# KoslickiLab/YACHT

Measured on AMD Instinct MI355X. Metric: ref-sketch containment queries/sec (yacht run), higher is better.
Workload: dtype u64

## Files before the change

### yacht_amd/csrc/yh_query.hip

```cpp
#include "yh_lookup.h"

#include <stdlib.h>
#include <string.h>

#include <algorithm>
#include <vector>

namespace {

constexpr int WAVE = 64;
constexpr int EXCL_PIECE_C = YH_EXCL_PIECE;

typedef u64 u64x2 __attribute__((ext_vector_type(2)));

__device__ __forceinline__ u32 xcd_remap(u32 bid, u32 nwg) {
    const u32 q = nwg >> 3, r = nwg & 7u;
    const u32 xcd = bid & 7u;
    const u32 base = (xcd < r) ? xcd * (q + 1) : r * (q + 1) + (xcd - r) * q;
    return base + (bid >> 3);
}

#ifndef YH_XCD_ATOMICS
#define YH_XCD_ATOMICS 0
#endif
__device__ __forceinline__ u32 xcc_id() { return (u32)__builtin_amdgcn_s_getreg((3 << 11) | 20) & 7u; }
__device__ __forceinline__ void count_add(u32* p, u32 v) {
#if YH_XCD_ATOMICS
    __hip_atomic_fetch_add(p, v, __ATOMIC_RELAXED, __HIP_MEMORY_SCOPE_WORKGROUP);
#else
    atomicAdd(p, v);
#endif
}
__device__ __forceinline__ u32 replica_of(u32 wg, u32 rep_mask) {
#if YH_XCD_ATOMICS
    return xcc_id() & rep_mask;
#else
    return wg & rep_mask;
#endif
}

struct FusedRun {
    u32* reps2;
    const u32* sizes;
    const u32* nshared;
    u32* n_excl;
    u32* n_match;
    u32* bits_out;
    const u32* rpo;
    uint4* work;
    u32* work_count;
    u32 work_refs;
};

__device__ __forceinline__ void append_pieces(bool in_subset, u32 j, u32 nshared_j, u32 rpo_j, uint4* __restrict__ work,
                                              u32* __restrict__ work_count, u32* lds ) {
    const u32 lane = threadIdx.x & 63u, wv = threadIdx.x >> 6, n_waves = blockDim.x >> 6;
    const u32 np = in_subset ? (nshared_j + (u32)EXCL_PIECE_C - 1u) / (u32)EXCL_PIECE_C : 0u;
    u32 v = np;
#pragma unroll
    for (int off = 1; off < 64; off <<= 1) {
        const u32 t = (u32)__shfl_up((int)v, off);
        if (lane >= (u32)off) v += t;
    }
    if (lane == 63) lds[wv] = v;
    __syncthreads();
    if (threadIdx.x == 0) {
        u32 total = 0;
        for (u32 q = 0; q < n_waves; ++q) total += lds[q];
        lds[n_waves] = total ? atomicAdd(work_count, total) : 0u;
    }
    __syncthreads();
    u32 at = lds[n_waves] + v - np;
    for (u32 q = 0; q < wv; ++q) at += lds[q];
    const u32 last = rpo_j + nshared_j;
    for (u32 i = 0; i < np; ++i) {
        const u32 first = rpo_j + i * (u32)EXCL_PIECE_C;
        work[at + i] = make_uint4(j, first, min(first + (u32)EXCL_PIECE_C, last), 0u);
    }
}

__device__ __forceinline__ void reduce_replicas_body(u32 wg, u32* lds, u32* __restrict__ reps, u32 R, u64 n,
                                                     u32* __restrict__ out, u8* __restrict__ mask,
                                                     u32* __restrict__ maskbits, u32* __restrict__ excl3,
                                                     const FusedRun& fused) {
    const u64 j = wg * (u64)blockDim.x + threadIdx.x;
    u32 acc = 0;
    u32 size_j = 0, nshared_j = 0, rpo_j = 0, rpo_end = 0;
    if (j < n && fused.reps2) {
        size_j = fused.sizes[j];
        nshared_j = fused.nshared[j];
        if (fused.work) { rpo_j = fused.rpo[j]; rpo_end = fused.rpo[j + 1]; }
    }
    if (j < n) {
        for (u32 r = 0; r < R; ++r) {
            acc += reps[(u64)r * n + j];
            reps[(u64)r * n + j] = 0;
        }
        out[j] = acc;
        if (mask) mask[j] = acc ? 1 : 0;
        if (excl3) { excl3[j] = 0; excl3[n + j] = 0; excl3[2 * n + j] = 0; }
        if (fused.reps2) {
            u32 acc2 = 0;
            for (u32 r = 0; r < R; ++r) {
                acc2 += fused.reps2[(u64)r * n + j];
                fused.reps2[(u64)r * n + j] = 0;
            }
            fused.n_match[j] = acc - acc2;
            if (fused.n_excl) fused.n_excl[j] = acc ? size_j - nshared_j : 0u;
        }
    }
    if (maskbits) {
        const u64 bal = __ballot(acc != 0);
        if ((threadIdx.x & 63) == 0 && (j >> 5) < ((n + 255) / 256) * 8) {
            maskbits[(j >> 5)] = (u32)bal;
            maskbits[(j >> 5) + 1] = (u32)(bal >> 32);
            if (fused.bits_out) {
                fused.bits_out[(j >> 5)] = (u32)bal;
                fused.bits_out[(j >> 5) + 1] = (u32)(bal >> 32);
            }
        }
    }
    if (fused.work) append_pieces(acc != 0 && j < fused.work_refs, (u32)j, rpo_end - rpo_j, rpo_j, fused.work, fused.work_count, lds);
}

__global__ void __launch_bounds__(256) k_reduce_replicas(u32* __restrict__ reps, u32 R, u64 n,
                                                         u32* __restrict__ out, u8* __restrict__ mask,
                                                         u32* __restrict__ maskbits, u32* __restrict__ excl3,
                                                         FusedRun fused) {
    __shared__ u32 lds[17];
    reduce_replicas_body(blockIdx.x, lds, reps, R, n, out, mask, maskbits, excl3, fused);
}

constexpr int FUSED_MAX_REPS = 16;
constexpr u32 FUSED_REPS_FORM1 = 8, FUSED_REPS_FORM2 = 8;
__device__ __forceinline__ u32 word_at(const u32* base, u32 byte_off) {
    return *reinterpret_cast<const u32*>(reinterpret_cast<const char*>(base) + byte_off);
}
template <int RPT, int G>
__device__ __forceinline__ void sum_replica_rows(const u32* set, u32 R, u64 n, const u32 (&off)[RPT], const bool (&ok)[RPT],
                                                 u32 (&acc)[RPT]) {
#pragma unroll 1
    for (u32 g = 0; g < R; g += (u32)G) {
        u32 t[RPT][G];
#pragma unroll
        for (u32 k = 0; k < (u32)G; ++k) {
            const u64 row = (u64)min(g + k, R - 1u) * n;
#pragma unroll
            for (int r = 0; r < RPT; ++r) t[r][k] = word_at(set + row, off[r]);
        }
#pragma unroll
        for (u32 k = 0; k < (u32)G; ++k)
#pragma unroll
            for (int r = 0; r < RPT; ++r) acc[r] += t[r][k] & ((ok[r] && g + k < R) ? ~0u : 0u);
    }
}
template <int RPT>
__device__ __forceinline__ void reduce_replicas_multi(u32 blk, u32* lds, u32* __restrict__ reps, u32 R, u64 n, u32* __restrict__ out,
                                                      u32* __restrict__ maskbits, const FusedRun& f) {
    const u32 lane = threadIdx.x & 63u, wv = threadIdx.x >> 6, n_waves = blockDim.x >> 6;
    const u64 j0 = (u64)blk * RPT * blockDim.x + threadIdx.x;
    u32 jj[RPT], off[RPT];
    bool ok[RPT];
    u32 acc[RPT], acc2[RPT], size_j[RPT], nsh[RPT], rpo0[RPT], rpo1[RPT];
#pragma unroll
    for (int r = 0; r < RPT; ++r) {
        ok[r] = j0 + (u64)r * blockDim.x < n;
        jj[r] = (u32)min(j0 + (u64)r * blockDim.x, n - 1);
        off[r] = jj[r] * 4u;
        acc[r] = acc2[r] = size_j[r] = nsh[r] = rpo0[r] = rpo1[r] = 0;
    }
    if (R >= 8u) sum_replica_rows<RPT, 8>(reps, R, n, off, ok, acc);
    else sum_replica_rows<RPT, 4>(reps, R, n, off, ok, acc);
#pragma unroll
    for (int r = 0; r < RPT; ++r) {
        if (acc[r]) {
            const u32 off1[1] = {off[r]};
            const bool ok1[1] = {true};
            u32 a2[1] = {0u};
            size_j[r] = f.sizes[jj[r]];
            nsh[r] = f.nshared[jj[r]];
            rpo0[r] = f.work ? f.rpo[jj[r]] : 0u;
            rpo1[r] = f.work ? f.rpo[jj[r] + 1u] : 0u;
            sum_replica_rows<1, 8>(f.reps2, R, n, off1, ok1, a2);
            acc2[r] = a2[0];
            for (u32 k = 0; k < R; ++k) (reps + (u64)k * n)[jj[r]] = 0;
            if (acc2[r])
                for (u32 k = 0; k < R; ++k) (f.reps2 + (u64)k * n)[jj[r]] = 0;
        }
    }
#pragma unroll
    for (int r = 0; r < RPT; ++r) {
        if (ok[r]) {
            out[jj[r]] = acc[r];
            f.n_match[jj[r]] = acc[r] - acc2[r];
            if (f.n_excl) f.n_excl[jj[r]] = acc[r] ? size_j[r] - nsh[r] : 0u;
        }
        const u64 bal = __ballot(acc[r] != 0);
        const u64 jr = j0 + (u64)r * blockDim.x;
        if (lane == 0 && (jr >> 5) < ((n + 255) / 256) * 8) {
            maskbits[(jr >> 5)] = (u32)bal;
            maskbits[(jr >> 5) + 1] = (u32)(bal >> 32);
            if (f.bits_out) { f.bits_out[(jr >> 5)] = (u32)bal; f.bits_out[(jr >> 5) + 1] = (u32)(bal >> 32); }
        }
    }
    if (!f.work) return;
    u32 np[RPT], mine = 0;
#pragma unroll
    for (int r = 0; r < RPT; ++r) {
        const bool in = acc[r] != 0 && jj[r] < f.work_refs;
        np[r] = in ? (rpo1[r] - rpo0[r] + (u32)EXCL_PIECE_C - 1u) / (u32)EXCL_PIECE_C : 0u;
        mine += np[r];
    }
    u32 v = mine;
#pragma unroll
    for (int off = 1; off < 64; off <<= 1) {
        const u32 t = (u32)__shfl_up((int)v, off);
        if (lane >= (u32)off) v += t;
    }
    if (lane == 63) lds[wv] = v;
    __syncthreads();
    if (threadIdx.x == 0) {
        u32 total = 0;
        for (u32 q = 0; q < n_waves; ++q) total += lds[q];
        lds[n_waves] = total ? atomicAdd(f.work_count, total) : 0u;
    }
    __syncthreads();
    u32 at = lds[n_waves] + v - mine;
    for (u32 q = 0; q < wv; ++q) at += lds[q];
#pragma unroll
    for (int r = 0; r < RPT; ++r) {
        const u32 last = rpo1[r];
        for (u32 i = 0; i < np[r]; ++i) {
            const u32 first = rpo0[r] + i * (u32)EXCL_PIECE_C;
            f.work[at + i] = make_uint4(jj[r], first, min(first + (u32)EXCL_PIECE_C, last), 0u);
        }
        at += np[r];
    }
}

__global__ void __launch_bounds__(256) k_excl_worklist(u64 n, const u32* __restrict__ maskbits, const u32* __restrict__ nshared,
                                                       const u32* __restrict__ rpo, uint4* __restrict__ work,
                                                       u32* __restrict__ work_count) {
    __shared__ u32 lds[17];
    const u64 j = blockIdx.x * (u64)blockDim.x + threadIdx.x;
    const bool in = j < n && ((maskbits[j >> 5] >> (j & 31u)) & 1u);
    append_pieces(in, (u32)j, in ? nshared[j] : 0u, in ? rpo[j] : 0u, work, work_count, lds);
}

__global__ void __launch_bounds__(256) k_ghost_bits(const u32* __restrict__ global_bits, const u32* __restrict__ src,
                                                    u64 ghost_begin, u64 n_ghost, u32* __restrict__ maskbits) {
    const u64 k = blockIdx.x * (u64)blockDim.x + threadIdx.x;
    bool on = false;
    if (k < n_ghost) {
        const u32 b = src[k];
        on = (global_bits[b >> 5] >> (b & 31u)) & 1u;
    }
    const u64 bal = __ballot(on);
    if ((threadIdx.x & 63) == 0 && (k & ~63ull) < n_ghost) {
        const u64 w = (ghost_begin + k) >> 5;
        maskbits[w] = (u32)bal;
        maskbits[w + 1] = (u32)(bal >> 32);
    }
}

__global__ void __launch_bounds__(256) k_range_mask(const u32* __restrict__ gathered, u32 n_ranks, u64 stride, u64 n,
                                                    const u32* __restrict__ sizes, const u32* __restrict__ nshared,
                                                    const u32* __restrict__ rpo, u32* __restrict__ maskbits,
                                                    u32* __restrict__ n_excl, uint4* __restrict__ work,
                                                    u32* __restrict__ work_count) {
    __shared__ u32 lds[17];
    const u64 j = blockIdx.x * (u64)blockDim.x + threadIdx.x;
    bool in = false;
    u32 size_j = 0, nshared_j = 0, rpo_j = 0, rpo_end = 0;
    if (j < n) {
        u32 w = 0;
        for (u32 r = 0; r < n_ranks; ++r) w |= gathered[(u64)r * stride + (j >> 5)];
        in = (w >> (j & 31u)) & 1u;
        size_j = sizes[j];
        nshared_j = nshared[j];
        if (work) { rpo_j = rpo[j]; rpo_end = rpo[j + 1]; }
        n_excl[j] = in ? size_j - nshared_j : 0u;
    }
    const u64 bal = __ballot(in);
    if ((threadIdx.x & 63) == 0) {
        maskbits[(j >> 5)] = (u32)bal;
        maskbits[(j >> 5) + 1] = (u32)(bal >> 32);
    }
// ... 305 lines not shown
                }
                wave_flush(hit, ctx, pend);
                if (c + np < 64) break;
                k += 64;
            }
        }
    }
}

constexpr int ST_LGNB = 11;
constexpr int ST_NB = 1 << ST_LGNB;

__global__ void __launch_bounds__(STREAM_THREADS, YH_STREAM_WAVES_PER_SIMD)
k_stream_lookup(const u32x4* __restrict__ deltas, const u64* __restrict__ hdr, u64 nblk,
                const u64* __restrict__ sample, u32 n_sample, const u64* __restrict__ wg_key, u32 sshift,
                StreamHit hit) {
    constexpr u32 WAVES = STREAM_THREADS / 64;
    __shared__ u32 S[ST_SLOTS];
    __shared__ u16 E[ST_NB];
    __shared__ u64x2 Q[WAVES][STREAM_WQ];
    __shared__ u32 INC[WAVES][STREAM_NB * INC_STRIDE];
    __shared__ u32 HB[WAVES][16];
    __shared__ u32 q_fill[WAVES];
    __shared__ u32 sbound[2];
    __shared__ u32 n_fit;
    __shared__ u32 tkey[STREAM_TSLOTS];
    __shared__ u32 tcnt[STREAM_TSLOTS];
    __shared__ u32 tcnt2[STREAM_TSLOTS];

    const u32 tid = threadIdx.x;
    if (hit.work_count && blockIdx.x == 0 && tid == 0) *hit.work_count = 0;
    if (hit.bad && *hit.bad == hit.bad_gen) return;
    const u32 wv = (u32)__builtin_amdgcn_readfirstlane((int)(tid >> 6));
    const u32 lid = xcd_remap(blockIdx.x, gridDim.x);
    const u64 per = (nblk + gridDim.x - 1) / gridDim.x;
    const u64 B0 = min((u64)lid * per, nblk), B1 = min(nblk, B0 + per);
    const WaveQ ctx{&q_fill[wv], Q[wv], lid, tkey, tcnt, tcnt2};
    if (B0 >= B1) return;
    u32x4 bufA[STREAM_PF], bufB[STREAM_PF];
    u64 hdrA = 0, hdrB = 0;
    const u64 first_sb = wv;
    if (first_sb * STREAM_NB < B1 - B0) load_group(deltas, hdr, B1, B0 + first_sb * STREAM_NB, bufA, hdrA);
    if (first_sb * STREAM_NB + STREAM_PF < B1 - B0) load_group(deltas, hdr, B1, B0 + first_sb * STREAM_NB + STREAM_PF, bufB, hdrB);
    if (wv < 2) {
        const u32 bnd = wave_bound(sample, n_sample, sshift, wg_key[lid + wv], wv == 1);
        if ((tid & 63u) == 0) sbound[wv] = bnd;
    }
    if (tid < WAVES) q_fill[tid] = 0;
    for (u32 k = tid; k < STREAM_TSLOTS; k += STREAM_THREADS) { tkey[k] = 0; tcnt[k] = 0; tcnt2[k] = 0; }
    __syncthreads();
    const u32 s0 = (u32)__builtin_amdgcn_readfirstlane((int)sbound[0]), s1 = (u32)__builtin_amdgcn_readfirstlane((int)sbound[1]);
    if (s0 >= s1) return;
    Pending pend;
    for (u32 sub = s0; sub < s1;) {
        u32 n = min((u32)ST_CAP, s1 - sub);
        if (sub != s0) __syncthreads();
        const u64 Klo = uniform_u64(sample[sub] >> sshift);
        if (tid == 0) n_fit = n;
        __syncthreads();
        for (u32 k = tid; k < n; k += STREAM_THREADS) {
            const u64 d = (sample[sub + k] >> sshift) - Klo;
            if (d > 0xfffffffeull) atomicMin(&n_fit, k);
            else S[k] = (u32)d;
        }
        __syncthreads();
        n = (u32)__builtin_amdgcn_readfirstlane((int)n_fit);
        for (u32 k = n + tid; k < n + ST_PAD; k += STREAM_THREADS) S[k] = 0xffffffffu;
        __syncthreads();
        const u32 span = (u32)__builtin_amdgcn_readfirstlane((int)S[n - 1]);
        const u64 Khi = Klo + span;
        const u32 dsh = (span >> ST_LGNB) ? (u32)(32 - __builtin_clz(span)) - ST_LGNB : 0u;
        for (u32 k = tid; k < n; k += STREAM_THREADS) {
            const u32 bk = S[k] >> dsh;
            const int bp = (k == 0) ? -1 : (int)(S[k - 1] >> dsh);
            for (int x = bp + 1; x <= (int)bk; ++x) E[x] = (u16)k;
            if (k == n - 1)
                for (u32 x = bk + 1; x < (u32)ST_NB; ++x) E[x] = (u16)n;
        }
        __syncthreads();
        const bool single = sub == s0 && n == s1 - s0;
        u64 bl0 = B0, bl1 = B1;
        if (!single) {
            u64 lo = B0, hi = B1;
            while (lo < hi) { const u64 mid = (lo + hi) >> 1; if (hdr[mid + 1] < Klo) lo = mid + 1; else hi = mid; }
            bl0 = lo;
            lo = bl0; hi = B1;
            while (lo < hi) { const u64 mid = (lo + hi) >> 1; if (hdr[mid] <= Khi) lo = mid + 1; else hi = mid; }
            bl1 = lo;
        }
        const u32 nb = (bl1 - bl0 >= 2ull * WAVES * STREAM_NB) ? (u32)STREAM_NB
                       : (u32)min((u64)STREAM_PF, max((bl1 - bl0) / WAVES, (u64)1));
        if (bl0 < bl1)
            stream_blocks(deltas, hdr, bl0, bl1, sub, n, Klo, Khi, dsh, S, E, INC[wv], HB[wv], hit, ctx, pend,
                          single && nb == (u32)STREAM_NB && first_sb * STREAM_NB < B1 - B0, nb, bufA, hdrA, bufB, hdrB);
        sub += n;
    }
    wave_flush(hit, ctx, pend);
    pending_count(hit, ctx, pend);
    __syncthreads();
    const u64 my = (u64)replica_of(lid, hit.rep_mask) * hit.n_refs;
    for (u32 k = tid; k < STREAM_TSLOTS; k += STREAM_THREADS)
        if (tkey[k]) {
            count_add(&hit.reps[my + tkey[k] - 1], tcnt[k]);
            if (hit.reps2 && tcnt2[k]) count_add(&hit.reps2[my + tkey[k] - 1], tcnt2[k]);
        }
}

__global__ void __launch_bounds__(256) k_overlap_bsearch(const u64* __restrict__ values,
                                                         const u64* __restrict__ offsets, u64 n_refs,
                                                         const u64* __restrict__ sample, u64 n_sample,
                                                         u32* __restrict__ overlap) {
    const u64 wave = (blockIdx.x * (u64)blockDim.x + threadIdx.x) / WAVE;
    const u64 n_waves = ((u64)gridDim.x * blockDim.x) / WAVE;
    const int lane = threadIdx.x & (WAVE - 1);
    for (u64 j = wave; j < n_refs; j += n_waves) {
        const u64 b = offsets[j], e = offsets[j + 1];
        u32 total = 0;
        for (u64 k0 = b; k0 < e; k0 += WAVE) {
            const u64 k = k0 + lane;
            bool hit = false;
            if (k < e) {
                const u64 h = values[k];
                u64 lo = 0, hi = n_sample;
                while (lo < hi) {
                    const u64 mid = (lo + hi) >> 1;
                    if (sample[mid] < h) lo = mid + 1; else hi = mid;
                }
                hit = (lo < n_sample) && (sample[lo] == h);
            }
            total += (u32)__popcll(__ballot(hit));
        }
        if (lane == 0) overlap[j] = total;
    }
}

struct TileLookup {
    const u64* sample;
    u64 n;
    YhDirView dv;
    const u32* filter;
    u64 filter_mul;
    const u64* po;
    const u32* pr;
    u32* reps;
    u32 rep_mask;
    u64 n_refs;
    u8* hit;
    u32* reps2;
    u32* work_count;
    const u32* bad;
    u32 bad_gen;
};
template <int U, int THREADS, int TBITS>
__device__ __forceinline__ void lookup_tile_body(u32 wg, u32* tkey, u32* tcnt, u32* tcnt2, const TileLookup& q) {
    constexpr u32 TSLOTS = 1u << TBITS;
    const u64* __restrict__ sample = q.sample;
    const u64 n = q.n;
    const YhDirView& dv = q.dv;
    const u32* __restrict__ filter = q.filter;
    if (q.work_count && wg == 0 && threadIdx.x == 0) *q.work_count = 0;
    u32* my = q.reps + (u64)replica_of(wg, q.rep_mask) * q.n_refs;
    u32* my2 = q.reps2 ? q.reps2 + (u64)replica_of(wg, q.rep_mask) * q.n_refs : nullptr;
    const u64 base = wg * (u64)(THREADS * U);
    u64 h[U];
    bool ok[U];
#pragma unroll
    for (int u = 0; u < U; ++u) {
        const u64 t = base + (u64)u * THREADS + threadIdx.x;
        h[u] = sample[min(t, n - 1)];
        ok[u] = t < n && h[u] <= dv.max_hash;
        if (!ok[u]) h[u] = 0;
    }
    if (q.bad && *q.bad == q.bad_gen) return;
    for (u32 k = threadIdx.x; k < TSLOTS; k += THREADS) { tkey[k] = 0; tcnt[k] = 0; tcnt2[k] = 0; }
    YhProbe<U> probe;
    u32 r[U];
    yh_probe_filter<U>(dv, filter, q.filter_mul, h, ok);
    yh_probe_request<U>(dv, h, ok, probe);
    __syncthreads();
    auto add = [&](u32 ref, bool shared) {
        const int slot = yh_hit_slot<TBITS>(tkey, ref);
        if (slot >= 0) {
            atomicAdd(&tcnt[slot], 1u);
            if (shared && my2) atomicAdd(&tcnt2[slot], 1u);
            return;
        }
        count_add(&my[ref], 1u);
        if (shared && my2) count_add(&my2[ref], 1u);
    };
#pragma unroll
    for (int u = 0; u < U; ++u) {
        r[u] = yh_probe_resolve<U>(dv, h, ok, probe, u);
        if (r[u] == YH_DIR_NONE) continue;
        if (!(r[u] & 0x80000000u)) {
            add(r[u], false);
        } else {
            const u32 gi = r[u] & 0x7fffffffu;
            if (q.hit) q.hit[gi] = 1;
            walk_holders(q.po, q.pr, gi, [&](u32 holder) { add(holder, true); });
        }
    }
    __syncthreads();
    for (u32 k = threadIdx.x; k < TSLOTS; k += THREADS)
        if (tkey[k]) {
            count_add(&my[tkey[k] - 1], tcnt[k]);
            if (my2 && tcnt2[k]) count_add(&my2[tkey[k] - 1], tcnt2[k]);
        }
}

template <int U, int THREADS, int TBITS>
__global__ void __launch_bounds__(THREADS) k_index_lookup_tile(const TileLookup q) {
    constexpr u32 TSLOTS = 1u << TBITS;
    __shared__ u32 tkey[TSLOTS];
    __shared__ u32 tcnt[TSLOTS];
    __shared__ u32 tcnt2[TSLOTS];
    lookup_tile_body<U, THREADS, TBITS>(blockIdx.x, tkey, tcnt, tcnt2, q);
}

constexpr u32 EXCL_PIECE = YH_EXCL_PIECE;
#ifndef YH_EXCL_U
#define YH_EXCL_U 4
#endif
constexpr int EXCL_U = YH_EXCL_U;
constexpr u32 EXCL_LDS_WORDS = 12288;

__device__ __forceinline__ u32 wave_sum(u32 v) {
#pragma unroll
    for (int off = 32; off >= 1; off >>= 1) v += (u32)__shfl_xor((int)v, off);
    return v;
}

template <class MaskWord>
__device__ __forceinline__ u32 others_in_subset(const uint4 rec, const uint4 recx, const u32* __restrict__ pr,
                                                const MaskWord& mword) {
    if (rec.w != 0xffffffffu) {
        const u32 hid[7] = {rec.x, rec.y, rec.z, recx.x, recx.y, recx.z, recx.w};
        u32 others = 0;
#pragma unroll
        for (int t = 0; t < 7; ++t) others += ((u32)t < rec.w) ? ((mword(hid[t] >> 5) >> (hid[t] & 31u)) & 1u) : 0u;
        return others;
    }
    u32 cnt = 0;
    const u32 q0 = rec.x, len = rec.y;
    for (u32 base = 0; base < len && cnt < 2; base += 8) {
        u32 h[8];
#pragma unroll
        for (int t = 0; t < 8; ++t) h[t] = pr[q0 + min(base + (u32)t, len - 1)];
#pragma unroll
        for (int t = 0; t < 8; ++t) cnt += (base + (u32)t < len) ? ((mword(h[t] >> 5) >> (h[t] & 31u)) & 1u) : 0u;
    }
    return cnt - 1u;
}

#ifndef YH_EXCL_GRID
#define YH_EXCL_GRID 2048
#endif
#ifndef YH_EXCL_RECX_ALWAYS
#define YH_EXCL_RECX_ALWAYS 0
#endif
constexpr int EXCL_PIECE_THREADS = YH_EXCL_PIECE_THREADS;
struct ExclPieces {
    const u32* work_count;
    const uint4* work;
    const u32* rpo;
    const u32* rg;
    const uint4* rrec;
    const uint4* rrecx;
    const u32* mult;
    const u64* po;
    u32 n_post;
    const u32* pr;
    const u32* maskbits;
    u32 n_mask_words;
    const u8* hit;
    u32* ex_e;
    u32* ex_m;
    u32* ovsh;
};
template <bool LDSMASK, int U>
__device__ __forceinline__ void excl_one_piece(const uint4 mine, const u32* lmask, const ExclPieces& q) {
    const u32 lane = threadIdx.x & 63u;
    const u32* __restrict__ rg = q.rg;
    const uint4* __restrict__ rrec = q.rrec;
    const uint4* __restrict__ rrecx = q.rrecx;
    const u32* __restrict__ mult = q.mult;
    const u32* __restrict__ pr = q.pr;
    const u8* __restrict__ hit = q.hit;
    const u32 n_post = q.n_post;
    auto mword = [&](u32 i) -> u32 { return LDSMASK ? lmask[i] : q.maskbits[i]; };
    const u32 r = mine.x;
    const u32 end = mine.z;
    u32 acc_e = 0, acc_m = 0, acc_o = 0;
    for (u32 k0 = mine.y; k0 < end; k0 += 64u * U) {
        u32 k[U];
        bool valid[U], in_s[U];
        uint4 rec[U], recx[U];
        u32 gi[U], mu[U];
#pragma unroll
        for (int u = 0; u < U; ++u) {
            k[u] = k0 + 64u * u + lane;
            valid[u] = k[u] < end;
            const u32 kc = min(k[u], n_post - 1);
            gi[u] = (hit || !rrec) ? rg[kc] : 0u;
            mu[u] = mult ? mult[kc] : 1u;
            if (rrec) rec[u] = rrec[kc];
            recx[u] = make_uint4(0u, 0u, 0u, 0u);
        }
        if (rrec) {
            bool more = YH_EXCL_RECX_ALWAYS != 0;
#pragma unroll
            for (int u = 0; u < U; ++u) more |= valid[u] && rec[u].w > 3u && rec[u].w != 0xffffffffu;
            if (__ballot(more)) {
#pragma unroll
                for (int u = 0; u < U; ++u) recx[u] = rrecx[min(k[u], n_post - 1)];
            }
        } else {
#pragma unroll
            for (int u = 0; u < U; ++u) {
                const u64 q0 = q.po[gi[u]], q1 = q.po[gi[u] + 1];
                rec[u] = make_uint4((u32)q0, (u32)(q1 - q0), 0u, 0xffffffffu);
            }
        }
#pragma unroll
        for (int u = 0; u < U; ++u) in_s[u] = hit && valid[u] && hit[gi[u]] != 0;
#pragma unroll
        for (int u = 0; u < U; ++u) {
            const bool e = valid[u] && others_in_subset(rec[u], recx[u], pr, mword) == 0;
            acc_e += e ? mu[u] : 0u;
            acc_m += (e && in_s[u]) ? 1u : 0u;
            acc_o += in_s[u] ? 1u : 0u;
        }
    }
    acc_e = wave_sum(acc_e);
    if (hit) { acc_m = wave_sum(acc_m); acc_o = wave_sum(acc_o); }
    if (lane == 0) {
        if (acc_e) atomicAdd(&q.ex_e[r], acc_e);
        if (hit && acc_m) atomicAdd(&q.ex_m[r], acc_m);
        if (hit && acc_o) atomicAdd(&q.ovsh[r], acc_o);
    }
}
__device__ __forceinline__ void stage_subset_bits(u32* lmask, const ExclPieces& q) {
    const uint4* src = reinterpret_cast<const uint4*>(q.maskbits);
    uint4* dst = reinterpret_cast<uint4*>(lmask);
    for (u32 i = threadIdx.x; i < q.n_mask_words / 4; i += blockDim.x) dst[i] = src[i];
    __syncthreads();
}

template <bool LDSMASK, int U = EXCL_U>
__device__ __forceinline__ void excl_pieces_body(u32 wg, u32 n_wgs, u32* lmask, const ExclPieces& q) {
    const u32 WPB = blockDim.x >> 6;
    const u32 n_work = *q.work_count;
    if (wg * WPB >= n_work) return;
    const u32 w0 = wg * WPB + (threadIdx.x >> 6);
    uint4 first_rec = make_uint4(0u, 0u, 0u, 0u);
    if (w0 < n_work) first_rec = q.work[w0];
    if (LDSMASK) stage_subset_bits(lmask, q);
    for (u32 w = w0; w < n_work; w += n_wgs * WPB)
        excl_one_piece<LDSMASK, U>((w == w0) ? first_rec : q.work[w], lmask, q);
}

template <bool LDSMASK>
__global__ void __launch_bounds__(EXCL_PIECE_THREADS) k_excl_pieces(const ExclPieces q) {
    extern __shared__ u32 lmask[];
    excl_pieces_body<LDSMASK>(blockIdx.x, gridDim.x, lmask, q);
}

struct StepFused {
    TileLookup look;   u32 look_wgs;
    u32* r_reps; u32 r_R; u64 r_n; u32* r_out; u32* r_maskbits; FusedRun r_fused; u32 red_wgs;
    ExclPieces excl;   u32 excl_wgs; u32 excl_lds;
};
template <int U, int THREADS, int TBITS>
__global__ void __launch_bounds__(THREADS, THREADS == 1024 ? 8 : 4) k_step_fused(const StepFused s) {
    extern __shared__ u32 smem[];
    constexpr u32 TSLOTS = 1u << TBITS;
    u32 b = blockIdx.x;
    if (b < s.excl_wgs) {
        if (s.excl_lds) excl_pieces_body<true, 2>(b, s.excl_wgs, smem, s.excl);
        else excl_pieces_body<false, 2>(b, s.excl_wgs, smem, s.excl);
        return;
    }
    b -= s.excl_wgs;
    if (b < s.red_wgs) {
        reduce_replicas_multi<4>(b, smem, s.r_reps, s.r_R, s.r_n, s.r_out, s.r_maskbits, s.r_fused);
        return;
    }
    b -= s.red_wgs;
    lookup_tile_body<U, THREADS, TBITS>(b, smem, smem + TSLOTS, smem + 2 * TSLOTS, s.look);
}

__global__ void k_excl_final(u64 n, const u8* __restrict__ mask, const u32* __restrict__ sizes,
                             const u32* __restrict__ nshared, const u32* __restrict__ overlap,
                             const u32* __restrict__ ex_e, const u32* __restrict__ ex_m,
                             const u32* __restrict__ ovsh, u32* __restrict__ out_e, u32* __restrict__ out_m,
                             uint4* __restrict__ hit16, u64 n_hit16) {
    const u64 j = blockIdx.x * (u64)blockDim.x + threadIdx.x;
    for (u64 i = j; i < n_hit16; i += (u64)gridDim.x * blockDim.x) hit16[i] = make_uint4(0, 0, 0, 0);
    if (j >= n) return;
    u32 e = 0, m = 0;
    if (mask[j]) {
        e = sizes[j] - nshared[j] + ex_e[j];
        m = overlap[j] - ovsh[j] + ex_m[j];
    }
    out_e[j] = e;
    out_m[j] = m;
}

inline u32 grid_for(u64 work_items, u32 block, u32 max_blocks = 16384) {
    u64 g = (work_items + block - 1) / block;
    if (g < 1) g = 1;
    if (g > max_blocks) g = max_blocks;
    return (u32)g;
}

}

int yh_q_check_sorted_host(const u64* v, u64 n) {
    for (u64 i = 1; i < n; ++i)
        if (!(v[i - 1] < v[i])) return YH_ERR_UNSORTED;
    return YH_OK;
}

static int ensure_reps(yh_db* db, u32& R) {
    const u64 N = db->n_refs;
    R = 32;
    while (R > 1 && (u64)R * N > (2u << 20)) R >>= 1;
    if (db->reps_cap < (u64)R * N) {
        YH_HIP(hipStreamSynchronize(db->stream));
        if (db->d_reps) { yh_dfree(db, db->d_reps); db->d_reps = nullptr; db->reps_cap = 0; }
        YH_HIP(hipMalloc((void**)&db->d_reps, 4 * (u64)R * N * sizeof(u32) + 16));
        YH_HIP(hipMemsetAsync(db->d_reps, 0, 4 * (u64)R * N * sizeof(u32) + 16, db->stream));
        db->reps_cap = (u64)R * N;
    }
    return YH_OK;
}
static int claim_hit_flags(yh_db* db) {
    if (!db->hit_clean && db->d_hit && db->n_shared)
        YH_HIP(hipMemsetAsync(db->d_hit, 0, db->n_shared + 15, db->stream));
    db->hit_clean = false;
    return YH_OK;
}

static ExclPieces excl_args(yh_db* db, const u32* work_count, const uint4* work, const u32* d_maskbits, const u8* d_hit,
                            u32* d_ex_e, u32* d_ex_m, u32* d_ovsh, bool sets) {
    const u32 words = (u32)(((db->n_refs + 255) / 256) * 8);
    return ExclPieces{work_count, work, db->d_rpo, db->d_rg, sets ? db->d_hrec : db->d_rrec, sets ? db->d_hrecx : db->d_rrecx,
                      sets ? db->d_hmult : nullptr, db->d_po, sets ? db->n_sets : (u32)db->n_postings, db->d_pr, d_maskbits,
                      words, d_hit, d_ex_e, d_ex_m, d_ovsh};
}
static void launch_excl_pieces(yh_db* db, const u32* d_maskbits, const u8* d_hit, u32* d_ex_e, u32* d_ex_m, u32* d_ovsh,
                               bool sets = false) {
    const ExclPieces q = excl_args(db, db->d_work_count, db->d_work, d_maskbits, d_hit, d_ex_e, d_ex_m, d_ovsh, sets);
    const u32 per_wg = EXCL_PIECE_THREADS / 64;
    const u32 grid = std::min<u32>((db->n_chunks + per_wg - 1) / per_wg, (u32)YH_EXCL_GRID);
    if (q.n_mask_words <= EXCL_LDS_WORDS)
        k_excl_pieces<true><<<grid, EXCL_PIECE_THREADS, q.n_mask_words * sizeof(u32), db->stream>>>(q);
    else
        k_excl_pieces<false><<<grid, EXCL_PIECE_THREADS, 0, db->stream>>>(q);
}

static int yh_q_overlap_stream(yh_db* db, const u64* d_sample, u64 n_sample, u32* d_overlap, bool flag_shared,
                               bool with_index, bool make_mask, u32* d_fused_excl = nullptr,
                               u32* d_fused_match = nullptr, u32* d_bits_out = nullptr) {
    hipStream_t st = db->stream;
    const u64 N = db->n_refs;
    const u64 nblk = db->slen / STREAM_BLOCK;
    static const u32 wgs_env = [] { const long long v = yh_tune_int("YH_STREAM_WGS", 512); return v > 0 ? (u32)v : 512u; }();
    u32 wgs = (u32)std::min<u64>(wgs_env, std::max<u64>(nblk / 2, 1));
    if (db->wg_key_n != wgs) {
        YH_HIP(hipStreamSynchronize(st));
        if (db->d_wg_key) { yh_dfree(db, db->d_wg_key); db->d_wg_key = nullptr; }
        YH_HIP(hipMalloc((void**)&db->d_wg_key, ((u64)wgs + 2) * sizeof(u64)));
        k_wg_key<<<(wgs + 256) / 256, 256, 0, st>>>(db->d_shdr, nblk, wgs, db->max_hash >> db->sshift, db->d_wg_key);
        db->wg_key_n = wgs;
    }
    u32 R;
    YH_TRY(ensure_reps(db, R));
    static const u32 r_env = (u32)yh_tune_int("YH_STREAM_REPS", YH_XCD_ATOMICS ? 8 : 4);
    while (R > 1 && R > r_env) R >>= 1;
    const bool fused = d_fused_excl != nullptr;
    const bool flags_too = flag_shared && db->has_index && !fused;
    if (flags_too) YH_TRY(claim_hit_flags(db));
    u32* const reps2 = db->d_reps + db->reps_cap;
    StreamHit sh{(u32)N, db->d_reps, R - 1, db->d_srec, flags_too ? db->d_hit : nullptr, db->d_g, (u32)db->n_shared,
                 fused ? reps2 : nullptr, d_sample, db->d_bad, db->bad_gen, db->d_work_count};
    yh_ring_record_begin(db, db->ev_overlap);
    k_stream_lookup<<<wgs, STREAM_THREADS, 0, st>>>(reinterpret_cast<const u32x4*>(db->d_sdelta), db->d_shdr, nblk, d_sample,
                                                    (u32)n_sample, db->d_wg_key, db->sshift, sh);
    yh_ring_record_end(db, db->ev_overlap);
    k_reduce_replicas<<<(u32)((N + 255) / 256), 256, 0, st>>>(
        db->d_reps, R, N, d_overlap, (make_mask && !fused) ? db->d_mask : nullptr, make_mask ? db->d_maskbits : nullptr,
        (with_index && !fused) ? db->d_excl_e : nullptr,
        fused ? FusedRun{reps2, db->d_sizes, db->d_nshared, db->range_local ? nullptr : d_fused_excl, d_fused_match, d_bits_out,
                         db->d_hpo, db->range_local ? nullptr : db->d_work, db->d_work_count,
                         (u32)(db->n_ghost ? db->ghost_begin : N)}
              : FusedRun{});
    YH_HIP(hipGetLastError());
    return YH_OK;
}

int yh_q_overlap(yh_db* db, const u64* d_sample, u64 n_sample, u32* d_overlap, bool flag_shared, bool make_mask) {
    if (!db->d_sdelta && db->n_hashes) { yh_set_error("this handle has no streaming layout (YH_DB_PAIRWISE_ONLY)"); return YH_ERR_UNSUPPORTED; }
    hipStream_t st = db->stream;
    const u64 N = db->n_refs;
    if (n_sample > 0xfffffff0ull) { yh_set_error("sample larger than 2^32-16 hashes"); return YH_ERR_INVALID_ARG; }
    const bool with_index = flag_shared && db->has_index;
    flag_shared = with_index && db->n_shared > 0;
    if (N == 0 || db->n_hashes == 0 || n_sample == 0) {
        YH_HIP(hipMemsetAsync(d_overlap, 0, std::max<u64>(N, 1) * sizeof(u32), st));
        if (flag_shared) { YH_HIP(hipMemsetAsync(db->d_hit, 0, db->n_shared + 15, st)); db->hit_clean = true; }
        if (with_index && N) YH_HIP(hipMemsetAsync(db->d_excl_e, 0, 3 * N * sizeof(u32), st));
        if (make_mask && N) {
            YH_HIP(hipMemsetAsync(db->d_mask, 0, N, st));
            YH_HIP(hipMemsetAsync(db->d_maskbits, 0, ((N + 255) / 256) * 32, st));
        }
        return YH_OK;
    }
    return yh_q_overlap_stream(db, d_sample, n_sample, d_overlap, flag_shared, with_index, make_mask);
}

int yh_q_run_fused(yh_db* db, const u64* d_sample, u64 n_sample, u32* d_overlap, u32* d_excl, u32* d_match, int phases,
                   u32* d_bits_out, const u32* d_global_bits, bool use_indexed) {
    static const bool off = yh_tune_flag("YH_NO_FUSED_RUN");
    if (!db->d_sdelta || !db->has_index || db->n_refs == 0 || db->n_hashes == 0 ||
        (db->n_postings && (!db->d_hrec || !db->d_hpo || !db->d_work)) || n_sample > 0xfffffff0ull)
        return 1;
    if (phases == 3 && (off || n_sample == 0)) return 1;
    hipStream_t st = db->stream;
    if (phases & 1) {
        if (n_sample == 0) {
            const u64 N = db->n_refs;
            YH_HIP(hipMemsetAsync(d_overlap, 0, N * sizeof(u32), st));
            YH_HIP(hipMemsetAsync(d_excl, 0, N * sizeof(u32), st));
            YH_HIP(hipMemsetAsync(d_match, 0, N * sizeof(u32), st));
            YH_HIP(hipMemsetAsync(db->d_maskbits, 0, ((N + 255) / 256) * 32, st));
            if (d_bits_out) YH_HIP(hipMemsetAsync(d_bits_out, 0, ((N + 255) / 256) * 32, st));
            if (db->d_work_count) YH_HIP(hipMemsetAsync(db->d_work_count, 0, sizeof(u32), st));
        } else if (use_indexed && db->has_dir && db->d_work && db->d_hrec && db->d_hpo) {
            const int rc = yh_q_overlap_indexed(db, d_sample, n_sample, d_overlap, true, d_excl, d_match, d_bits_out, true);
            if (rc != 2) return rc == YH_OK ? YH_ERR_UNSUPPORTED : rc;
        } else {
            YH_TRY(yh_q_overlap_stream(db, d_sample, n_sample, d_overlap, true, true, true, d_excl, d_match, d_bits_out));
        }
    }
    if (phases & 2) {
        yh_ring_record_begin(db, db->ev_excl);
        if (db->n_ghost && d_global_bits)
            k_ghost_bits<<<(u32)((db->n_ghost + 255) / 256), 256, 0, st>>>(d_global_bits, db->d_ghost_src, db->ghost_begin,
                                                                        db->n_ghost, db->d_maskbits);
        if (db->n_chunks)
            launch_excl_pieces(db, db->d_maskbits, nullptr, d_excl, nullptr, nullptr, true);
        yh_ring_record_end(db, db->ev_excl);
    }
    YH_HIP(hipGetLastError());
    return YH_OK;
}

static bool fused_possible(const yh_db* db, const u32* d_fused_excl, bool for_exclusive) {
    static const bool fused_off = yh_tune_flag("YH_NO_FUSED_RUN");
    return d_fused_excl && for_exclusive && db->d_work && db->d_hrec && db->d_hpo && !fused_off;
}

int yh_q_range_finish(yh_db* db, const u32* d_gathered, u32 n_ranks, u64 stride_words, u32* d_excl) {
    if (!db->has_index || db->n_refs == 0) return YH_OK;
    hipStream_t st = db->stream;
    const u64 N = db->n_refs;
    const bool sets = db->n_postings && db->d_hrec && db->d_hpo && db->d_work;
    yh_ring_record_begin(db, db->ev_excl);
    k_range_mask<<<(u32)((N + 255) / 256), 256, 0, st>>>(d_gathered, n_ranks, stride_words, N, db->d_sizes, db->d_nshared,
                                                          sets ? db->d_hpo : nullptr, db->d_maskbits, d_excl,
                                                          sets ? db->d_work : nullptr, db->d_work_count);
    if (sets && db->n_chunks) launch_excl_pieces(db, db->d_maskbits, nullptr, d_excl, nullptr, nullptr, true);
    yh_ring_record_end(db, db->ev_excl);
    YH_HIP(hipGetLastError());
    return YH_OK;
}

int yh_q_overlap_indexed(yh_db* db, const u64* d_sample, u64 n_sample, u32* d_overlap, bool for_exclusive,
                         u32* d_fused_excl, u32* d_fused_match, u32* d_bits_out, bool lookup_half_only) {
    if (!db->has_dir || !db->has_index) {
        yh_set_error("this handle has no directory of its distinct hashes (YH_DB_NO_DIRECTORY, or no index)");
        return YH_ERR_UNSUPPORTED;
    }
    hipStream_t st = db->stream;
    const u64 N = db->n_refs;
    if (N == 0) return YH_OK;
    u32 R;
    YH_TRY(ensure_reps(db, R));
    static const u32 ri_env = (u32)yh_tune_int("YH_INDEX_REPS", 0);
    static const long tile_env = (long)yh_tune_int("YH_INDEX_TILE", -1);
    const YhTileShape shape = tile_env == 256 ? yh_tile_shape(0) : tile_env == 1 ? yh_tile_shape(1) : tile_env == 2 ? yh_tile_shape(2)
                              : tile_env == 4 ? yh_tile_shape(3) : yh_tile_shape_for(n_sample);
    const u32 r_want = ri_env ? ri_env : 4u;
    while (R > 1 && R > r_want) R >>= 1;
    const bool fused = fused_possible(db, d_fused_excl, for_exclusive);
    if (for_exclusive && db->n_shared && !fused) YH_TRY(claim_hit_flags(db));
    u32* const reps1 = db->d_reps;
    u32* const reps2 = reps1 + db->reps_cap;
    yh_ring_record_begin(db, db->ev_overlap);
    u8* const d_hitflags = (for_exclusive && db->n_shared && !fused) ? db->d_hit : nullptr;
    u32* const d_reps2 = fused ? reps2 : nullptr;
    if (n_sample && db->n_distinct) {
        const TileLookup q{d_sample, n_sample, yh_dir_view(db), shape.filter ? yh_filter_of(db) : nullptr, db->filter_mul, db->d_po, db->d_pr,
                           reps1, R - 1, N, d_hitflags, d_reps2, db->d_work_count, db->d_bad, db->bad_gen};
        switch (shape.form) {
        case 0: k_index_lookup_tile<1, 256, 8><<<shape.tiles(n_sample), 256, 0, st>>>(q); break;
        case 1: k_index_lookup_tile<1, 1024, 10><<<shape.tiles(n_sample), 1024, 0, st>>>(q); break;
        case 2: k_index_lookup_tile<2, 1024, 10><<<shape.tiles(n_sample), 1024, 0, st>>>(q); break;
        default: k_index_lookup_tile<4, 1024, 10><<<shape.tiles(n_sample), 1024, 0, st>>>(q); break;
        }
    }
    else if (fused && db->d_work_count)
        YH_HIP(hipMemsetAsync(db->d_work_count, 0, sizeof(u32), st));
    yh_ring_record_end(db, db->ev_overlap);
    k_reduce_replicas<<<(u32)((N + 255) / 256), 256, 0, st>>>(
        reps1, R, N, d_overlap, (for_exclusive && !fused) ? db->d_mask : nullptr,
        for_exclusive ? db->d_maskbits : nullptr, (for_exclusive && !fused) ? db->d_excl_e : nullptr,
        fused ? FusedRun{reps2, db->d_sizes, db->d_nshared, db->range_local ? nullptr : d_fused_excl, d_fused_match, d_bits_out,
                         db->d_hpo, db->range_local ? nullptr : db->d_work, db->d_work_count,
                         (u32)(db->n_ghost ? db->ghost_begin : N)}
              : FusedRun{});
    if (fused && !lookup_half_only) {
        yh_ring_record_begin(db, db->ev_excl);
        if (db->n_chunks) launch_excl_pieces(db, db->d_maskbits, nullptr, d_fused_excl, nullptr, nullptr, true);
        yh_ring_record_end(db, db->ev_excl);
    }
    YH_HIP(hipGetLastError());
    return fused ? 2 : YH_OK;
}

bool yh_q_step_fused_ok(const yh_db* db, u64 n_sample) {
    return db->has_dir && db->has_index && db->d_cbkt && fused_possible(db, reinterpret_cast<const u32*>(db), true) &&
           db->n_chunks && !db->n_ghost && n_sample >= 1 && n_sample <= 0xfffffff0ull &&
           db->n_refs < (1ull << 30);
}
int yh_q_step_fused(yh_db* db, const u64* d_sample, u64 n_sample, u32* d_overlap, u32* d_excl, u32* d_match) {
    hipStream_t st = db->stream;
    const u64 N = db->n_refs;
    u32 R;
    YH_TRY(ensure_reps(db, R));
    const YhTileShape shape = d_sample ? yh_tile_shape_for(n_sample) : yh_tile_shape(0);
    static const u32 reps_env = (u32)std::max<long long>(yh_tune_int("YH_FUSED_REPS", 0), 0);
    static const u32 fused_reps[3] = {4u, FUSED_REPS_FORM1, FUSED_REPS_FORM2};
    const u32 r_want = std::min<u32>(reps_env ? reps_env : fused_reps[shape.form], (u32)FUSED_MAX_REPS);
    while (R > 1 && R > r_want) R >>= 1;
    const u32 threads = shape.threads, waves = threads / 64, tslots = 1u << shape.tbits;
    StepFused s{};
    u32 lds_words = 3 * tslots;
    if (db->pend_excl >= 0) {
        const int c = db->pend_excl;
        s.excl = excl_args(db, db->ctx_count[c], db->ctx_work[c], db->ctx_bits[c], nullptr, db->pend_excl_out, nullptr, nullptr, true);
        static const u32 wgs_env = (u32)yh_tune_int("YH_FUSED_EXCL_WGS", 0);
        s.excl_wgs = std::min<u32>((db->n_chunks + waves - 1) / waves, 4096u / waves);
        if (wgs_env) s.excl_wgs = std::max<u32>(std::min<u32>(wgs_env, s.excl_wgs), 1u);
        s.excl_lds = s.excl.n_mask_words <= EXCL_LDS_WORDS ? 1u : 0u;
        if (s.excl_lds) lds_words = std::max(lds_words, s.excl.n_mask_words);
    }
    if (db->pend_red >= 0) {
        const int c = db->pend_red;
        u32* const reps1 = db->d_reps + (u64)(db->pend_red_parity & 1) * 2 * db->reps_cap;
        s.r_reps = reps1;
        s.r_R = (u32)db->pend_red_parity >> 1;
        s.r_n = N;
        s.r_out = db->pend_red_out[0];
        s.r_maskbits = db->ctx_bits[c];
        s.r_fused = FusedRun{reps1 + db->reps_cap, db->d_sizes, db->d_nshared, db->pend_red_out[1], db->pend_red_out[2], nullptr,
                             db->d_hpo, db->ctx_work[c], db->ctx_count[c], (u32)N};
        s.red_wgs = (u32)((N + 4ull * threads - 1) / (4ull * threads));
    }
    int c_new = -1;
    if (d_sample) {
        c_new = (int)(db->pipe_k % 3);
        const int parity = (int)(db->pipe_k & 1);
        u32* const reps1 = db->d_reps + (u64)parity * 2 * db->reps_cap;
        s.look = TileLookup{d_sample, n_sample, yh_dir_view(db), shape.filter ? yh_filter_of(db) : nullptr, db->filter_mul, db->d_po, db->d_pr,
                            reps1, R - 1, N, nullptr, reps1 + db->reps_cap, db->ctx_count[c_new], nullptr, 0u};
        s.look_wgs = shape.tiles(n_sample);
    }
    const u32 total = s.excl_wgs + s.red_wgs + s.look_wgs;
    if (total) {
        if (d_sample) yh_ring_record_begin(db, db->ev_overlap);
        switch (shape.form) {
        case 2: k_step_fused<2, 1024, 10><<<total, 1024, lds_words * sizeof(u32), st>>>(s); break;
        case 1: k_step_fused<1, 1024, 10><<<total, 1024, lds_words * sizeof(u32), st>>>(s); break;
        default: k_step_fused<1, 256, 8><<<total, 256, lds_words * sizeof(u32), st>>>(s); break;
        }
        if (d_sample) yh_ring_record_end(db, db->ev_overlap);
        YH_HIP(hipGetLastError());
    }
    db->pend_excl = db->pend_red;
    db->pend_excl_out = db->pend_red >= 0 ? db->pend_red_out[1] : nullptr;
    db->pend_red = c_new;
    if (d_sample) {
        db->pend_red_parity = (int)((db->pipe_k & 1) | (R << 1));
        db->pend_red_out[0] = d_overlap;
        db->pend_red_out[1] = d_excl;
        db->pend_red_out[2] = d_match;
        db->pipe_last_ctx = c_new;
        ++db->pipe_k;
    }
    return YH_OK;
}

int yh_q_overlap_bsearch(yh_db* db, const u64* d_sample, u64 n_sample, u32* d_overlap) {
    if (!db->d_values) { yh_set_error("yh_overlap_bsearch needs a handle created with YH_DB_KEEP_CSR"); return YH_ERR_UNSUPPORTED; }
    hipStream_t st = db->stream;
    const u64 N = db->n_refs;
    YH_HIP(hipMemsetAsync(d_overlap, 0, std::max<u64>(N, 1) * sizeof(u32), st));
    if (N == 0) return YH_OK;
    k_overlap_bsearch<<<grid_for(N * WAVE, 256, 8192), 256, 0, st>>>(db->d_values, db->d_offsets, N, d_sample, n_sample,
                                                                     d_overlap);
    YH_HIP(hipGetLastError());
    return YH_OK;
}

int yh_q_exclusive(yh_db* db, const u8* d_mask, const u64* d_sample, u64 n_sample, const u32* d_overlap,
                   u32* d_excl, u32* d_match, const u32* d_maskbits) {
    (void)d_sample; (void)n_sample;
    if (!db->has_index) { yh_set_error("this handle was created with YH_DB_NO_INDEX"); return YH_ERR_UNSUPPORTED; }
    if (db->flags & YH_DB_PAIRWISE_ONLY) { yh_set_error("this handle holds posting lists only"); return YH_ERR_UNSUPPORTED; }
    hipStream_t st = db->stream;
    const u64 N = db->n_refs;
    if (N == 0) return YH_OK;
    yh_ring_record_begin(db, db->ev_excl);
    if (!d_maskbits) {
        k_mask_bits<<<(u32)((N + 255) / 256), 256, 0, st>>>(d_mask, N, db->d_maskbits);
        d_maskbits = db->d_maskbits;
    }
    if (db->n_shared && db->n_chunks) {
        YH_HIP(hipMemsetAsync(db->d_work_count, 0, sizeof(u32), st));
        k_excl_worklist<<<(u32)((N + 255) / 256), 256, 0, st>>>(N, d_maskbits, db->d_nshared, db->d_rpo, db->d_work, db->d_work_count);
        launch_excl_pieces(db, d_maskbits, db->d_hit, db->d_excl_e, db->d_excl_m, db->d_ovsh);
    }
    const bool clean_hit = db->d_hit && db->n_shared;
    k_excl_final<<<grid_for(N, 256, 1u << 22), 256, 0, st>>>(
        N, d_mask, db->d_sizes, db->d_nshared, d_overlap, db->d_excl_e, db->d_excl_m, db->d_ovsh, d_excl, d_match,
        clean_hit ? reinterpret_cast<uint4*>(db->d_hit) : nullptr, clean_hit ? (db->n_shared + 15) / 16 : 0);
    if (clean_hit) db->hit_clean = true;
    yh_ring_record_end(db, db->ev_excl);
    YH_HIP(hipGetLastError());
    return YH_OK;
}
```

Measured before the change: 2.812 billion.

## Add grid-stride persistent lookup tiles sharing one LDS hit table per workgroup

Adds a grid-stride variant of the sample lookup tile body, so one workgroup processes several tiles while reusing its LDS hot-reference counters and flushes them to global replicas only once. In the fused step kernel the lookup workgroup count is capped at 512 for forms 1 and 2, which turns striding on whenever there are more tiles than that. The standalone index lookup only strides when an env var sets a smaller grid. The aim is fewer global atomic flushes and less per-tile table setup, at the cost of fewer workgroups to hide latency.

```diff
diff --git a/yacht_amd/csrc/yh_query.hip b/yacht_amd/csrc/yh_query.hip
--- a/yacht_amd/csrc/yh_query.hip
+++ b/yacht_amd/csrc/yh_query.hip
@@ -133,6 +133,8 @@
 
 constexpr int FUSED_MAX_REPS = 16;
 constexpr u32 FUSED_REPS_FORM1 = 8, FUSED_REPS_FORM2 = 8;
+constexpr u32 FUSED_TILES_FORM1 = 1, FUSED_TILES_FORM2 = 1;
+constexpr u32 FUSED_LOOK_WGS_MAX = 512;
 __device__ __forceinline__ u32 word_at(const u32* base, u32 byte_off) {
     return *reinterpret_cast<const u32*>(reinterpret_cast<const char*>(base) + byte_off);
 }
@@ -744,7 +746,7 @@
     u32 bad_gen;
 };
 template <int U, int THREADS, int TBITS>
-__device__ __forceinline__ void lookup_tile_body(u32 wg, u32* tkey, u32* tcnt, u32* tcnt2, const TileLookup& q) {
+__device__ __forceinline__ void lookup_one_tile(u32 wg, u32* tkey, u32* tcnt, u32* tcnt2, const TileLookup& q) {
     constexpr u32 TSLOTS = 1u << TBITS;
     const u64* __restrict__ sample = q.sample;
     const u64 n = q.n;
@@ -800,13 +802,81 @@
         }
 }
 
-template <int U, int THREADS, int TBITS>
-__global__ void __launch_bounds__(THREADS) k_index_lookup_tile(const TileLookup q) {
+template <bool B> struct TileFirst { static constexpr bool value = B; };
+template <int U, int THREADS, int TBITS, bool ONE_TRIP = false>
+__device__ __forceinline__ void lookup_tile_body(u32 wg, u32 n_wgs, u32* tkey, u32* tcnt, u32* tcnt2, const TileLookup& q) {
+    if constexpr (ONE_TRIP) { lookup_one_tile<U, THREADS, TBITS>(wg, tkey, tcnt, tcnt2, q); return; }
+    constexpr u32 TSLOTS = 1u << TBITS;
+    const u64* __restrict__ sample = q.sample;
+    const u64 n = q.n;
+    const YhDirView& dv = q.dv;
+    const u32* __restrict__ filter = q.filter;
+    if (q.work_count && wg == 0 && threadIdx.x == 0) *q.work_count = 0;
+    u32* my = q.reps + (u64)replica_of(wg, q.rep_mask) * q.n_refs;
+    u32* my2 = q.reps2 ? q.reps2 + (u64)replica_of(wg, q.rep_mask) * q.n_refs : nullptr;
+    auto add = [&](u32 ref, bool shared) {
+        const int slot = yh_hit_slot<TBITS>(tkey, ref);
+        if (slot >= 0) {
+            atomicAdd(&tcnt[slot], 1u);
+            if (shared && my2) atomicAdd(&tcnt2[slot], 1u);
+            return;
+        }
+        count_add(&my[ref], 1u);
+        if (shared && my2) count_add(&my2[ref], 1u);
+    };
+    auto tile_pass = [&](u64 base, auto first) __attribute__((always_inline)) {
+        u64 h[U];
+        bool ok[U];
+#pragma unroll
+        for (int u = 0; u < U; ++u) {
+            const u64 t = base + (u64)u * THREADS + threadIdx.x;
+            h[u] = sample[min(t, n - 1)];
+            ok[u] = t < n && h[u] <= dv.max_hash;
+            if (!ok[u]) h[u] = 0;
+        }
+        if constexpr (decltype(first)::value) {
+            if (q.bad && *q.bad == q.bad_gen) return false;
+            for (u32 k = threadIdx.x; k < TSLOTS; k += THREADS) { tkey[k] = 0; tcnt[k] = 0; tcnt2[k] = 0; }
+        }
+        YhProbe<U> probe;
+        u32 r[U];
+        yh_probe_filter<U>(dv, filter, q.filter_mul, h, ok);
+        yh_probe_request<U>(dv, h, ok, probe);
+        if constexpr (decltype(first)::value) __syncthreads();
+#pragma unroll
+        for (int u = 0; u < U; ++u) {
+            r[u] = yh_probe_resolve<U>(dv, h, ok, probe, u);
+            if (r[u] == YH_DIR_NONE) continue;
+            if (!(r[u] & 0x80000000u)) {
+                add(r[u], false);
+            } else {
+                const u32 gi = r[u] & 0x7fffffffu;
+                if (q.hit) q.hit[gi] = 1;
+                walk_holders(q.po, q.pr, gi, [&](u32 holder) { add(holder, true); });
+            }
+        }
+        return true;
+    };
+    if (!tile_pass(wg * (u64)(THREADS * U), TileFirst<true>{})) return;
+    const u32 n_tiles = (u32)((n + (u64)(THREADS * U) - 1) / (u64)(THREADS * U));
+#pragma unroll 1
+    for (u32 tile = wg + n_wgs; tile < n_tiles; tile += n_wgs)
+        tile_pass(uniform64(tile * (u64)(THREADS * U)), TileFirst<false>{});
+    __syncthreads();
+    for (u32 k = threadIdx.x; k < TSLOTS; k += THREADS)
+        if (tkey[k]) {
+            count_add(&my[tkey[k] - 1], tcnt[k]);
+            if (my2 && tcnt2[k]) count_add(&my2[tkey[k] - 1], tcnt2[k]);
+        }
+}
+
+template <int U, int THREADS, int TBITS, bool STRIDE = false>
+__global__ void __launch_bounds__(THREADS, (STRIDE && THREADS == 1024 && U <= 2) ? 8 : 1) k_index_lookup_tile(const TileLookup q) {
     constexpr u32 TSLOTS = 1u << TBITS;
     __shared__ u32 tkey[TSLOTS];
     __shared__ u32 tcnt[TSLOTS];
     __shared__ u32 tcnt2[TSLOTS];
-    lookup_tile_body<U, THREADS, TBITS>(blockIdx.x, tkey, tcnt, tcnt2, q);
+    lookup_tile_body<U, THREADS, TBITS, !STRIDE>(blockIdx.x, gridDim.x, tkey, tcnt, tcnt2, q);
 }
 
 constexpr u32 EXCL_PIECE = YH_EXCL_PIECE;
@@ -962,7 +1032,7 @@
     u32* r_reps; u32 r_R; u64 r_n; u32* r_out; u32* r_maskbits; FusedRun r_fused; u32 red_wgs;
     ExclPieces excl;   u32 excl_wgs; u32 excl_lds;
 };
-template <int U, int THREADS, int TBITS>
+template <int U, int THREADS, int TBITS, bool STRIDE = false>
 __global__ void __launch_bounds__(THREADS, THREADS == 1024 ? 8 : 4) k_step_fused(const StepFused s) {
     extern __shared__ u32 smem[];
     constexpr u32 TSLOTS = 1u << TBITS;
@@ -978,7 +1048,7 @@
         return;
     }
     b -= s.red_wgs;
-    lookup_tile_body<U, THREADS, TBITS>(b, smem, smem + TSLOTS, smem + 2 * TSLOTS, s.look);
+    lookup_tile_body<U, THREADS, TBITS, !STRIDE>(b, s.look_wgs, smem, smem + TSLOTS, smem + 2 * TSLOTS, s.look);
 }
 
 __global__ void k_excl_final(u64 n, const u8* __restrict__ mask, const u32* __restrict__ sizes,
@@ -1195,11 +1265,22 @@
     if (n_sample && db->n_distinct) {
         const TileLookup q{d_sample, n_sample, yh_dir_view(db), shape.filter ? yh_filter_of(db) : nullptr, db->filter_mul, db->d_po, db->d_pr,
                            reps1, R - 1, N, d_hitflags, d_reps2, db->d_work_count, db->d_bad, db->bad_gen};
-        switch (shape.form) {
-        case 0: k_index_lookup_tile<1, 256, 8><<<shape.tiles(n_sample), 256, 0, st>>>(q); break;
-        case 1: k_index_lookup_tile<1, 1024, 10><<<shape.tiles(n_sample), 1024, 0, st>>>(q); break;
-        case 2: k_index_lookup_tile<2, 1024, 10><<<shape.tiles(n_sample), 1024, 0, st>>>(q); break;
-        default: k_index_lookup_tile<4, 1024, 10><<<shape.tiles(n_sample), 1024, 0, st>>>(q); break;
+        static const u32 look_env = (u32)std::max<long long>(yh_tune_int("YH_INDEX_LOOK_WGS", 0), 0);
+        const u32 grid = look_env ? std::min<u32>(look_env, shape.tiles(n_sample)) : shape.tiles(n_sample);
+        if (grid < shape.tiles(n_sample)) {
+            switch (shape.form) {
+            case 0: k_index_lookup_tile<1, 256, 8, true><<<grid, 256, 0, st>>>(q); break;
+            case 1: k_index_lookup_tile<1, 1024, 10, true><<<grid, 1024, 0, st>>>(q); break;
+            case 2: k_index_lookup_tile<2, 1024, 10, true><<<grid, 1024, 0, st>>>(q); break;
+            default: k_index_lookup_tile<4, 1024, 10, true><<<grid, 1024, 0, st>>>(q); break;
+            }
+        } else {
+            switch (shape.form) {
+            case 0: k_index_lookup_tile<1, 256, 8><<<grid, 256, 0, st>>>(q); break;
+            case 1: k_index_lookup_tile<1, 1024, 10><<<grid, 1024, 0, st>>>(q); break;
+            case 2: k_index_lookup_tile<2, 1024, 10><<<grid, 1024, 0, st>>>(q); break;
+            default: k_index_lookup_tile<4, 1024, 10><<<grid, 1024, 0, st>>>(q); break;
+            }
         }
     }
     else if (fused && db->d_work_count)
@@ -1261,20 +1342,33 @@
         s.red_wgs = (u32)((N + 4ull * threads - 1) / (4ull * threads));
     }
     int c_new = -1;
+    bool stride = false;
     if (d_sample) {
         c_new = (int)(db->pipe_k % 3);
         const int parity = (int)(db->pipe_k & 1);
         u32* const reps1 = db->d_reps + (u64)parity * 2 * db->reps_cap;
         s.look = TileLookup{d_sample, n_sample, yh_dir_view(db), shape.filter ? yh_filter_of(db) : nullptr, db->filter_mul, db->d_po, db->d_pr,
                             reps1, R - 1, N, nullptr, reps1 + db->reps_cap, db->ctx_count[c_new], nullptr, 0u};
-        s.look_wgs = shape.tiles(n_sample);
+        static const u32 look_env = (u32)std::max<long long>(yh_tune_int("YH_FUSED_LOOK_WGS", 0), 0);
+        static const u32 tiles_env = (u32)std::max<long long>(yh_tune_int("YH_FUSED_TILES", 0), 0);
+        static const u32 fused_tiles[3] = {1u, FUSED_TILES_FORM1, FUSED_TILES_FORM2};
+        const u32 tiles = shape.tiles(n_sample), per_wg = (tiles_env && shape.form) ? tiles_env : fused_tiles[shape.form];
+        s.look_wgs = tiles;
+        if (shape.form) s.look_wgs = look_env ? std::min<u32>(look_env, tiles) : std::min<u32>((tiles + per_wg - 1) / per_wg, FUSED_LOOK_WGS_MAX);
+        stride = s.look_wgs < tiles;
     }
     const u32 total = s.excl_wgs + s.red_wgs + s.look_wgs;
     if (total) {
         if (d_sample) yh_ring_record_begin(db, db->ev_overlap);
         switch (shape.form) {
-        case 2: k_step_fused<2, 1024, 10><<<total, 1024, lds_words * sizeof(u32), st>>>(s); break;
-        case 1: k_step_fused<1, 1024, 10><<<total, 1024, lds_words * sizeof(u32), st>>>(s); break;
+        case 2:
+            if (stride) k_step_fused<2, 1024, 10, true><<<total, 1024, lds_words * sizeof(u32), st>>>(s);
+            else k_step_fused<2, 1024, 10><<<total, 1024, lds_words * sizeof(u32), st>>>(s);
+            break;
+        case 1:
+            if (stride) k_step_fused<1, 1024, 10, true><<<total, 1024, lds_words * sizeof(u32), st>>>(s);
+            else k_step_fused<1, 1024, 10><<<total, 1024, lds_words * sizeof(u32), st>>>(s);
+            break;
         default: k_step_fused<1, 256, 8><<<total, 256, lds_words * sizeof(u32), st>>>(s); break;
         }
         if (d_sample) yh_ring_record_end(db, db->ev_overlap);
```

Result: no change. 2.803 billion (-0.3%).
